# ermongroup/TEOChat

Hardware: AMD Instinct MI355X
Metric: end-to-end tokens/sec (prefill+decode), T=8 frames, LLaMA-2-7B (higher is better)
Workload: dtype bf16; 1 GPU; C3: T=8 frames 224x224 -> CLIP-ViT-L/14 (23 layers) -> mlp2x_gelu -> splice of a 128-token prompt (L=2168) -> LLaMA-2-7B prefill -> 256 forced greedy tokens; value = generated tokens / total time; frames=8, sequence_len=2168, parallelism=dp1 (1 conversation per GPU, no collective), weights=random N(0,0.02^2) at LLaMA-2-7B / ViT-L/14 shapes

## Files before the change

### teochat_amd/_lib.py

```python
import ctypes as C
import os
import threading

HERE = os.path.dirname(os.path.abspath(__file__))
LIB_PATH = os.path.join(HERE, "libteo_hip.so")

TEO_F32, TEO_BF16, TEO_F16 = 0, 1, 2
ACT_NONE, ACT_GELU_ERF, ACT_QUICK_GELU = 0, 1, 2
GEMM_SWIGLU16, GEMM_FORCE_SIMPLE, GEMM_WTILED, GEMM_SWIGLU8, GEMM_F16 = 1, 2, 4, 8, 16
GEMV_W13 = 32
ATTN_FORCE_SIMPLE = 1
INT32_MIN = -(2 ** 31)


class TeoLibraryError(RuntimeError):
    pass


class TeoError(RuntimeError):
    pass


class AttnArgs(C.Structure):
    _fields_ = [("q", C.c_void_p), ("k", C.c_void_p), ("v", C.c_void_p), ("vt", C.c_void_p), ("o", C.c_void_p),
# ... 218 lines not shown
    _fields_ = [("d_next", C.c_void_p), ("n_states", C.c_int), ("vocab", C.c_int), ("d_state", C.c_void_p), ("fallback_token", C.c_longlong)]


_SIGS_GUIDE = {
    "teo_guide_sizeof": (C.c_size_t, []),
    "teo_guide_mask": (C.c_int, [C.c_void_p, C.c_longlong, C.c_int, C.POINTER(Guide), C.c_void_p]),
    "teo_guide_advance": (C.c_int, [C.POINTER(Guide), C.c_void_p, C.c_int, C.c_void_p]),
    "teo_llama_decode_step_guided": (C.c_int, [C.POINTER(LlamaDesc), C.POINTER(DecodeState), C.POINTER(Guide), C.c_void_p, C.c_size_t, C.c_void_p]),
    "teo_llama_decode_graph_create_guided": (C.c_int, [C.POINTER(LlamaDesc), C.POINTER(DecodeState), C.POINTER(Guide), C.c_void_p, C.c_size_t,
                                                       C.c_void_p, C.POINTER(C.c_void_p)]),
    "teo_llama_decode_stream_step_guided": (C.c_int, [C.POINTER(LlamaDesc), C.POINTER(DecodeStreamState), C.POINTER(Guide), C.c_void_p, C.c_size_t,
                                                      C.c_void_p]),
    "teo_llama_decode_stream_graph_create_guided": (C.c_int, [C.POINTER(LlamaDesc), C.POINTER(DecodeStreamState), C.POINTER(Guide), C.c_void_p,
                                                              C.c_size_t, C.c_void_p, C.POINTER(C.c_void_p)]),
}
EXPORTS_GUIDE = tuple(_SIGS_GUIDE.keys())


class Share(C.Structure):
    _fields_ = [("d_lead", C.c_void_p), ("d_rows", C.c_void_p)]


_SIGS_SHARE = {
    "teo_share_sizeof": (C.c_size_t, []),
    "teo_attn_decode_shared": (C.c_int, [C.c_void_p] * 9 + [C.c_int] * 4 + [C.c_float, C.c_int, C.c_int, C.c_longlong, C.c_longlong,
                                                                             C.c_longlong, C.c_void_p, C.c_void_p, C.c_void_p]),
    "teo_attn_decode_chunk": (C.c_int, [C.c_int] * 5 + [C.c_void_p]),
    "teo_llama_decode_stream_step_shared": (C.c_int, [C.POINTER(LlamaDesc), C.POINTER(DecodeStreamState), C.POINTER(Share), C.POINTER(Guide),
                                                      C.c_void_p, C.c_size_t, C.c_void_p]),
    "teo_llama_decode_stream_graph_create_shared": (C.c_int, [C.POINTER(LlamaDesc), C.POINTER(DecodeStreamState), C.POINTER(Share),
                                                              C.POINTER(Guide), C.c_void_p, C.c_size_t, C.c_void_p, C.POINTER(C.c_void_p)]),
}
EXPORTS_SHARE = tuple(_SIGS_SHARE.keys())
_lib = None


def load():
    global _lib
    if _lib is not None:
        return _lib
    import torch
    if not os.path.exists(LIB_PATH):
        raise TeoLibraryError(
            f"{LIB_PATH} not found: the HIP library is required (no CPU fallback). Build it with "
            "`python -c \"import __graft_entry__ as g; g.build()\"` or `make -C teochat_amd/csrc`.")
    try:
        lib = C.CDLL(LIB_PATH)
    except OSError as e:
        raise TeoLibraryError(f"cannot load {LIB_PATH}: {e}") from e
    for name, (res, args) in list(_SIGS.items()) + list(_SIGS_PREFIX.items()) + list(_SIGS_SCORE.items()) + list(_SIGS_GUIDE.items()) \
            + list(_SIGS_SHARE.items()):
        try:
            fn = getattr(lib, name)
        except AttributeError as e:
            raise TeoLibraryError(f"{LIB_PATH} does not export {name}; rebuild it") from e
        fn.restype = res
        fn.argtypes = args
    if lib.teo_version() != ABI_VERSION:
        raise TeoLibraryError(f"ABI version mismatch: library {lib.teo_version()}, binding {ABI_VERSION}; rebuild {LIB_PATH}")
    mirrors = {"teo_vit_desc": VitDesc, "teo_proj_desc": ProjDesc, "teo_llama_desc": LlamaDesc, "teo_decode_state": DecodeState,
               "teo_decode_batch_state": DecodeBatchState, "teo_attn_args": AttnArgs, "teo_verify_state": VerifyState,
               "teo_decode_stream_state": DecodeStreamState}
    for name, cls in mirrors.items():
        want = lib.teo_sizeof(name.encode())
        if want != C.sizeof(cls):
            raise TeoLibraryError(f"struct layout mismatch: {name} is {want} bytes in {LIB_PATH}, {C.sizeof(cls)} in this binding; rebuild")
    if lib.teo_guide_sizeof() != C.sizeof(Guide):
        raise TeoLibraryError(f"struct layout mismatch: teo_guide is {lib.teo_guide_sizeof()} bytes in {LIB_PATH}, {C.sizeof(Guide)} in this binding; rebuild")
    if lib.teo_share_sizeof() != C.sizeof(Share):
        raise TeoLibraryError(f"struct layout mismatch: teo_share is {lib.teo_share_sizeof()} bytes in {LIB_PATH}, {C.sizeof(Share)} in this binding; rebuild")
    _lib = lib
    return lib


class Tune:

    def __init__(self):
        self._lib = load()
        self.ptr = self._lib.teo_tune_create()
        if not self.ptr:
            raise TeoError("teo_tune_create failed")

    def try_set(self, key, value):
        key = key if isinstance(key, bytes) else key.encode()
# ... 75 lines not shown
```

### teochat_amd/csrc/abi.hip

```cpp
#include <stdarg.h>

#include <new>

#include "runtime.h"

namespace teo {

static thread_local char g_err[512] = "";

thread_local const char* g_last_kernel = "";
void note_kernel(const char* name) { g_last_kernel = name; }

void set_error(const char* fmt, ...) {
    va_list ap;
    va_start(ap, fmt);
    vsnprintf(g_err, sizeof(g_err), fmt, ap);
    va_end(ap);
}

int device_cu_count() {
    static int cached[64];
    int dev = 0;
    if (hipGetDevice(&dev) != hipSuccess) return 0;
    if (dev >= 0 && dev < 64 && cached[dev] > 0) return cached[dev];
    hipDeviceProp_t p;
    const int cus = hipGetDeviceProperties(&p, dev) == hipSuccess ? p.multiProcessorCount : 0;
    if (dev >= 0 && dev < 64 && cus > 0) cached[dev] = cus;
    return cus;
}

int lds_attr_once(const void* kernel, int bytes, unsigned long long* mask, const char* what) {
    int dev = 0;
    if (hipGetDevice(&dev) != hipSuccess) dev = 0;
    const unsigned long long bit = 1ull << (dev & 63);
    if (__atomic_load_n(mask, __ATOMIC_RELAXED) & bit) return TEO_OK;
    const hipError_t e = hipFuncSetAttribute(kernel, hipFuncAttributeMaxDynamicSharedMemorySize, bytes);
    if (e != hipSuccess) { set_error("%s: hipFuncSetAttribute(%d bytes of LDS): %s", what, bytes, hipGetErrorString(e)); return TEO_ERR_HIP; }
// ... 681 lines not shown
        if (e != hipSuccess) return hip_fail(e, "hipGraphLaunch");
    }
    return TEO_OK;
}

int teo_graph_destroy(teo_graph* g) {
    if (!g) return TEO_OK;
    if (g->exec) (void)hipGraphExecDestroy(g->exec);
    if (g->graph) (void)hipGraphDestroy(g->graph);
    delete g;
    return TEO_OK;
}

size_t teo_attn_decode_workspace_bytes(int heads, int head_dim, int max_seq, int batch) {
    if (!(heads > 0 && head_dim > 0 && max_seq > 0 && batch > 0)) return 0;
    return attn_decode_ws_bytes(heads, head_dim, max_seq, batch);
}

int teo_attn_decode(const void* q, void* k_cache, void* v_cache, void* vt_cache, const float* rope_cos, const float* rope_sin,
                    void* out, float* partials, const int* d_pos, int max_seq, int heads, int kv_heads, int head_dim, float scale,
                    int dtype, int batch, long long q_stride, long long cache_stride, long long o_stride, teo_stream_t s) {
    ENTER();
    NEED_DT(dtype);
    TEO_CHECK_ARG(batch >= 1 && heads > 0 && kv_heads > 0 && heads % kv_heads == 0 && head_dim > 0 && max_seq > 0,
                  "teo_attn_decode: batch %d heads %d kv_heads %d head_dim %d max_seq %d", batch, heads, kv_heads, head_dim, max_seq);
    NEED(q, "q"); NEED(k_cache, "k_cache"); NEED(v_cache, "v_cache"); NEED(out, "out"); NEED(partials, "partials"); NEED(d_pos, "d_pos");
    TEO_CHECK_ARG((rope_cos == nullptr) == (rope_sin == nullptr), "teo_attn_decode: rope_cos and rope_sin go together");
    AttnBatch bt;
    bt.batch = batch; bt.q_stride = q_stride; bt.cache_stride = cache_stride; bt.o_stride = o_stride;
    return attn_decode(q, k_cache, v_cache, vt_cache, rope_cos, rope_sin, out, partials, d_pos, max_seq, heads, kv_heads, head_dim,
                       scale, dtype, ST(s), bt);
}

size_t teo_attn_verify_workspace_bytes(int heads, int head_dim, int max_seq, int rows) {
    if (!(heads > 0 && head_dim > 0 && max_seq > 0 && rows > 0)) return 0;
    return attn_decode_ws_bytes(heads, head_dim, max_seq, rows);
}

int teo_attn_verify(const void* qkv, void* k_cache, void* v_cache, void* vt_cache, const float* rope_cos, const float* rope_sin,
                    void* out, float* partials, const int* d_pos, int max_seq, int heads, int kv_heads, int head_dim, float scale,
                    int dtype, int rows, long long q_stride, teo_stream_t s) {
    ENTER();
    NEED_DT(dtype);
    TEO_CHECK_ARG(rows >= 1 && rows <= TEO_MAX_DECODE_BATCH && heads > 0 && kv_heads > 0 && heads % kv_heads == 0 && max_seq >= rows,
                  "teo_attn_verify: rows %d (1..%d) heads %d kv_heads %d max_seq %d", rows, TEO_MAX_DECODE_BATCH, heads, kv_heads, max_seq);
    TEO_CHECK_ARG(head_dim > 0, "teo_attn_verify: head_dim %d", head_dim);
    NEED(qkv, "qkv"); NEED(k_cache, "k_cache"); NEED(v_cache, "v_cache"); NEED(out, "out"); NEED(partials, "partials"); NEED(d_pos, "d_pos");
    NEED(rope_cos, "rope_cos"); NEED(rope_sin, "rope_sin");
    TEO_CHECK_ARG(q_stride >= (long long)(heads + 2 * kv_heads) * head_dim && q_stride % (dtype == TEO_F32 ? 4 : 8) == 0,
                  "teo_attn_verify: q_stride %lld (whole [q|k|v] rows, 16-byte aligned)", q_stride);
    return attn_verify(qkv, k_cache, v_cache, vt_cache, rope_cos, rope_sin, out, partials, d_pos, max_seq, heads, kv_heads, head_dim,
                       scale, dtype, rows, q_stride, ST(s));
}

int teo_cross_entropy(const float* logits, long long ld, const long long* labels, float* loss_row, float* out, int rows, int vocab,
                      long long ignore_index, teo_stream_t s) {
    ENTER();
    TEO_CHECK_ARG(rows >= 0 && vocab > 0 && ld >= vocab, "teo_cross_entropy: rows %d vocab %d ld %lld", rows, vocab, ld);
    NEED(out, "out");
    if (rows) { NEED(logits, "logits"); NEED(labels, "labels"); NEED(loss_row, "loss_row"); }
    return cross_entropy(logits, ld, labels, loss_row, out, rows, vocab, ignore_index, ST(s));
}

int teo_preprocess_frames(const unsigned char* src, void* out, int T, int H, int W, int S, const float* mean, const float* stdv,
                          int dtype, teo_stream_t s) {
    ENTER();
// ... 52 lines not shown
```

### teochat_amd/csrc/attention.hip

```cpp
#include "common.h"
#include "ops.h"

namespace teo {

typedef __attribute__((ext_vector_type(8))) short bf16x8;
typedef __attribute__((ext_vector_type(4))) float f32x4;
typedef __attribute__((ext_vector_type(4))) unsigned int u32x4;

template <typename T>
__global__ __launch_bounds__(64) void attn_simple_kernel(teo_attn_args a) {
    extern __shared__ __attribute__((aligned(16))) float sm[];
    float* qs = sm;
    float* sc = sm + a.head_dim;
    const int i = blockIdx.x, h = blockIdx.y, b = blockIdx.z, lane = threadIdx.x;
    const int hk = h / (a.heads / a.kv_heads);
    const int hd = a.head_dim;
    const T* q = (const T*)a.q + b * a.q_bs + h * a.q_hs + (long long)i * a.q_rs;
    const T* k = (const T*)a.k + b * a.k_bs + hk * a.k_hs;
    const T* v = (const T*)a.v + b * a.v_bs + hk * a.v_hs;
    for (int d = lane; d < hd; d += 64) qs[d] = Elem<T>::ld(q + d);
    __syncthreads();
    const int lim = a.causal ? min(a.kv_len, i + (a.kv_len - a.q_len) + 1) : a.kv_len;
    float mx = -INFINITY;
    for (int j = lane; j < lim; j += 64) {
// ... 294 lines not shown
    for (int i = 0; i < SPL; ++i)
        if (DEC_CHUNK >= 64 || lane + 64 * i < DEC_CHUNK) pstrip[wid][lane + 64 * i] = Elem<T>::round(sv[i]);
    float acc[VE];
#pragma unroll
    for (int e = 0; e < VE; ++e) acc[e] = 0.f;
#pragma unroll
    for (int i = 0; i < NI; ++i) {
        const float p = pstrip[wid][wid * KPW + i * RPI + grp];
        if constexpr (ROPE) {
            float vf[VE];
            Cvt16<T>::cvt(vr[i], vf);
            if (kw0 + i * RPI + grp >= pos) {
#pragma unroll
                for (int e = 0; e < VE; ++e) vf[e] = vnew[e];
            }
#pragma unroll
            for (int e = 0; e < VE; ++e) acc[e] = fmaf(p, vf[e], acc[e]);
        } else {
            attn_pv_fma<T>(vr[i], p, acc);
        }
    }
#pragma unroll
    for (int e = 0; e < VE; ++e) acc[e] = cross_group_sum<LPR>(acc[e]);
    if (grp == 0) {
#pragma unroll
        for (int e = 0; e < VE; ++e) obuf[wid][sub * VE + e] = acc[e];
    }
    __syncthreads();
    for (int d = tid; d < HD; d += 256) out[2 + d] = obuf[0][d] + obuf[1][d] + obuf[2][d] + obuf[3][d];
    if (tid == 0) { out[0] = mx; out[1] = sum; }
}

template <typename T>
__device__ __forceinline__ void attn_merge_records(const float* __restrict__ pb, int stride, int nact, int hd_log2, T* __restrict__ o_row,
                                                   float* w , float* red , float* accs ) {
    const int tid = threadIdx.x, lane = tid & 63, wid = tid >> 6;
    const bool on = tid < 512;
    const int hd = 1 << hd_log2;
    const int G = 512 >> hd_log2;
    const int g = on ? tid >> hd_log2 : 0, d = tid & (hd - 1);
    constexpr int NB = 12;
    float v0[NB];
#pragma unroll
    for (int i = 0; i < NB; ++i) v0[i] = pb[(unsigned)(min(g + i * G, nact - 1) * stride + 2 + d)];
    float m0 = -INFINITY, l0 = 0.f;
    if (tid < nact) { m0 = pb[(unsigned)(tid * stride)]; l0 = pb[(unsigned)(tid * stride + 1)]; }
    float M = wave_max(m0);
    if (lane == 0 && on) red[wid] = M;
    __syncthreads();
    M = fmaxf(fmaxf(red[0], red[1]), fmaxf(red[2], red[3]));
    const float w0 = (m0 == -INFINITY) ? 0.f : expf(m0 - M);
    if (tid < 256) w[tid] = w0;
    float L = wave_sum(l0 * w0);
    if (lane == 0 && on) red[8 + wid] = L;
    __syncthreads();
    const float inv = 1.0f / ((red[8] + red[9]) + (red[10] + red[11]));
    float a = 0.f;
#pragma unroll
    for (int i = 0; i < NB; ++i) {
        const float t = v0[i] * w[min(g + i * G, 255)];
        a += (g + i * G < nact) ? t : 0.f;
    }
    for (int s0 = g + NB * G; s0 < nact; s0 += 8 * G) {
        float v[8];
#pragma unroll
        for (int i = 0; i < 8; ++i) v[i] = pb[(unsigned)(min(s0 + i * G, nact - 1) * stride + 2 + d)];
#pragma unroll
        for (int i = 0; i < 8; ++i) {
            const float t = v[i] * w[min(s0 + i * G, 255)];
            a += (s0 + i * G < nact) ? t : 0.f;
        }
    }
    if (on) accs[tid] = a;
    __syncthreads();
    if (on && g == 0) {
        float t = 0.f;
        for (int k = 0; k < G; ++k) t += accs[d + k * hd];
        Elem<T>::st(o_row + d, t * inv);
    }
}

template <typename T>
__global__ __launch_bounds__(512) void attn_decode_combine_kernel(const int* __restrict__ d_pos, const float* __restrict__ part,
                                                                  T* __restrict__ o, int hd_log2, int nsplit, int chunk_log2,
                                                                  long long o_stride) {
    __shared__ float w[256];
    __shared__ float red[16];
    __shared__ float accs[512];
    const int pos = d_pos[blockIdx.y];
    const int h = blockIdx.x;
    const int hd = 1 << hd_log2;
    const int stride = hd + 2;
    part += (long long)blockIdx.y * gridDim.x * nsplit * stride;
    o += (long long)blockIdx.y * o_stride;
    if (pos < 0) {
        if ((int)threadIdx.x < hd) Elem<T>::st(o + h * hd + threadIdx.x, 0.f);
        return;
    }
    const float* pb = part + (long long)h * nsplit * stride;
    const int nact = min(nsplit, (pos + (1 << chunk_log2)) >> chunk_log2);
    attn_merge_records<T>(pb, stride, nact, hd_log2, o + h * hd, w, red, accs);
}

template <typename T, int LPR, int DEC_CHUNK, bool ROPE, int AW_WAVES, bool PROBE = false>
__global__ __launch_bounds__(AW_WAVES * 64) void attn_decode_whole_kernel(const T* __restrict__ q, T* __restrict__ kc, T* __restrict__ vc,
                                                                          T* __restrict__ vtc, const float* __restrict__ cs,
                                                                          const float* __restrict__ sn, T* __restrict__ o,
                                                                          const int* __restrict__ d_pos, int S_max, int heads, int kv_heads,
                                                                          float scale, AttnBatch bt) {
    constexpr int VE = Cvt16<T>::N;
    constexpr int HD = LPR * VE;
    constexpr int RPI = 64 / LPR;
    constexpr int KPQ = DEC_CHUNK / 4;
    constexpr int NI = KPQ / RPI;
    constexpr int SPL = (DEC_CHUNK + 63) / 64;
    constexpr int STRIDE = HD + 2;
    extern __shared__ __attribute__((aligned(16))) float aw_lds[];
    float* sc = aw_lds + (threadIdx.x >> 6) * DEC_CHUNK;
    float* rec = aw_lds + AW_WAVES * DEC_CHUNK;
    {
        const long long bz = blockIdx.y;
        q += bz * bt.q_stride;
        kc += bz * bt.cache_stride;
        vc += bz * bt.cache_stride;
        if (vtc) vtc += bz * bt.cache_stride;
        d_pos += bz;
        o += bz * bt.o_stride;
    }
    const int h = blockIdx.x, tid = threadIdx.x, lane = tid & 63, wid = tid >> 6;
    const int hk = (heads == kv_heads) ? h : h / (heads / kv_heads);
    const int kv_len = *d_pos + 1;
    if (kv_len <= 0) {
        if (!PROBE && tid < HD) Elem<T>::st(o + h * HD + tid, 0.f);
        return;
// ... 142 lines not shown
        }
        mx = wave_max(mx);
        float sum = 0.f;
#pragma unroll
        for (int i = 0; i < SPL; ++i) { sv[i] = expf(sv[i] - mx); sum += sv[i]; }
        sum = wave_sum(sum);
        __builtin_amdgcn_wave_barrier();
#pragma unroll
        for (int i = 0; i < SPL; ++i)
            if (DEC_CHUNK >= 64 || lane + 64 * i < DEC_CHUNK) sc[lane + 64 * i] = Elem<T>::round(sv[i]);
        __builtin_amdgcn_wave_barrier();
        float ot[VE];
        TEO_AW_PV(r0, 0, ot)
        TEO_AW_ISSUE(r0, kb, cn, 0, nlive)
        TEO_AW_PV(r1, 1, ot)
        TEO_AW_ISSUE(r1, kb, cn, 1, nlive)
        TEO_AW_PV(r2, 2, ot)
        TEO_AW_ISSUE(r2, kb, cn, 2, nlive)
        TEO_AW_PV(r3, 3, ot)
        TEO_AW_ISSUE(r3, kb, cn, 3, nlive)
        __builtin_amdgcn_wave_barrier();
        float* rc = rec + (long long)c * STRIDE;
        if (grp == 0) {
#pragma unroll
            for (int e = 0; e < VE; ++e) rc[2 + sub * VE + e] = ot[e];
        }
        if (lane == 0) { rc[0] = mx; rc[1] = sum; }
    }
#undef TEO_AW_ISSUE
#undef TEO_AW_SCORES
#undef TEO_AW_PV
    __syncthreads();
    float* w = rec + (long long)nact * STRIDE;
    attn_merge_records<T>(rec, STRIDE, nact, __builtin_ctz((unsigned)HD), o + h * HD, w, w + 256, w + 272);
}

size_t attn_decode_ws_bytes(int heads, int hd, int S_max, int batch) {
    const int nsplit = cdiv(S_max, 32);
    return (size_t)batch * heads * nsplit * (hd + 2) * sizeof(float);
}

template <typename T, int LPR>
static void attn_decode_launch(const void* q, void* kc, void* vc, void* vtc, const float* cs, const float* sn, void* o,
                               float* part, const int* d_pos, int S_max, int heads, int kv_heads, int hd, float scale,
                               int nsplit, int chunk, bool rope, AttnBatch bt, hipStream_t st) {
    dim3 grid(heads, nsplit, bt.batch);
#define TEO_PART(CH, RP)                                                                                              \
    TEO_KLAUNCH((attn_decode_partial_kernel<T, LPR, CH, RP>), grid, 256, 0, st, d_pos, (T*)kc, (T*)vc, (const T*)q, S_max, heads, kv_heads,      \
                                                                     nsplit, (T*)vtc, cs, sn, part, scale, bt)
#define TEO_PART_R(CH) if (rope) { TEO_PART(CH, true); } else { TEO_PART(CH, false); }
    if constexpr (32 / 4 >= 64 / LPR) {
        if (chunk == 32) { TEO_PART_R(32) } else if (chunk == 64) { TEO_PART_R(64) } else if (chunk == 256) { TEO_PART_R(256) } else { TEO_PART_R(128) }
    } else if constexpr (64 / 4 >= 64 / LPR) {
        if (chunk == 64) { TEO_PART_R(64) } else if (chunk == 256) { TEO_PART_R(256) } else { TEO_PART_R(128) }
    } else {
        if (chunk == 256) { TEO_PART_R(256) } else { TEO_PART_R(128) }
    }
#undef TEO_PART_R
#undef TEO_PART
    prof_bump(1);
    TEO_KLAUNCH((attn_decode_combine_kernel<T>), dim3(heads, bt.batch), 512, 0, st, d_pos, part, (T*)o, __builtin_ctz((unsigned)hd), nsplit,
                __builtin_ctz((unsigned)chunk), bt.o_stride);
    prof_bump(-1);
}

template <typename T, int LPR, int NW>
static int attn_whole_launch_t(const void* q, void* kc, void* vc, void* vtc, const float* cs, const float* sn, void* o, const int* d_pos,
                               int S_max, int heads, int kv_heads, float scale, int chunk, bool rope, AttnBatch bt, size_t lds, hipStream_t st) {
    constexpr int RPI = 64 / LPR;
    dim3 grid(heads, bt.batch);
#define TEO_AW(CH, RP)                                                                                                          \
    {                                                                                                                           \
        static unsigned long long attr_mask = 0;                                                                                \
        if (lds > 48 * 1024) if (int e = lds_attr_once(reinterpret_cast<const void*>(&attn_decode_whole_kernel<T, LPR, CH, RP, NW>), 96 * 1024, &attr_mask, "attn_decode_whole")) return e; \
        TEO_KLAUNCH((attn_decode_whole_kernel<T, LPR, CH, RP, NW>), grid, NW * 64, lds, st, (const T*)q, (T*)kc, (T*)vc, (T*)vtc, cs, sn, \
                    (T*)o, d_pos, S_max, heads, kv_heads, scale, bt);                                                           \
    }
#define TEO_AW_R(CH) { if (rope) TEO_AW(CH, true) else TEO_AW(CH, false) }
    if (chunk == 128) { if constexpr (128 / 4 / RPI >= 1 && 128 / 4 / RPI <= 8) TEO_AW_R(128) else return TEO_ERR_UNSUPPORTED; }
    else if (chunk == 64) { if constexpr (64 / 4 / RPI >= 1 && 64 / 4 / RPI <= 8) TEO_AW_R(64) else return TEO_ERR_UNSUPPORTED; }
    else if (chunk == 32) { if constexpr (32 / 4 / RPI >= 1 && 32 / 4 / RPI <= 8) TEO_AW_R(32) else return TEO_ERR_UNSUPPORTED; }
    else return TEO_ERR_UNSUPPORTED;
#undef TEO_AW_R
#undef TEO_AW
    note_kernel("attn_decode_whole");
    TEO_LAUNCH_CHECK("attn_decode_whole");
    return TEO_OK;
}

static int attn_whole_launch(const void* q, void* kc, void* vc, void* vtc, const float* cs, const float* sn, void* o, const int* d_pos, int S_max,
                             int heads, int kv_heads, int hd, float scale, int chunk, int lpr, int dtype, AttnBatch bt, size_t lds, hipStream_t st) {
    const bool rope = cs != nullptr;
#define TEO_AWL(TT, LL) return attn_whole_launch_t<TT, LL, 8>(q, kc, vc, vtc, cs, sn, o, d_pos, S_max, heads, kv_heads, scale, chunk, rope, bt, lds, st)
    if (dtype == TEO_F32) {
        switch (lpr) { case 4: TEO_AWL(float, 4); case 8: TEO_AWL(float, 8); case 16: TEO_AWL(float, 16); case 32: TEO_AWL(float, 32); default: return TEO_ERR_UNSUPPORTED; }
    }
    if (dtype == TEO_F16) {
        switch (lpr) { case 4: TEO_AWL(f16_t, 4); case 8: TEO_AWL(f16_t, 8); case 16: TEO_AWL(f16_t, 16); case 32: TEO_AWL(f16_t, 32); default: return TEO_ERR_UNSUPPORTED; }
    }
    switch (lpr) { case 4: TEO_AWL(bf16_t, 4); case 8: TEO_AWL(bf16_t, 8); case 16: TEO_AWL(bf16_t, 16); case 32: TEO_AWL(bf16_t, 32); default: return TEO_ERR_UNSUPPORTED; }
#undef TEO_AWL
}

struct AttnDecodePlan {
    int lpr, chunk, nsplit;
    bool ok;
    bool whole;
    int cw;
    size_t lds_whole;
};
static AttnDecodePlan attn_decode_plan(int batch, int heads, int hd, int S_max, int dtype) {
    AttnDecodePlan p;
    int chunk = tune().attn_chunk ? tune().attn_chunk : (batch > 1 ? 128 : 64);
    const int esz = dtype == TEO_F32 ? 4 : 2;
    const int lpr = hd * esz / 16;
    if (chunk / 4 < 64 / lpr) chunk = 4 * (64 / lpr);
    if (chunk != 32 && chunk != 64 && chunk != 128 && chunk != 256) chunk = 128;
    while (chunk < 256 && cdiv(S_max, chunk) > 256) chunk *= 2;
    p.lpr = lpr; p.chunk = chunk; p.nsplit = cdiv(S_max, chunk);
    p.ok = !(p.nsplit > 256 || (hd * esz) % 16 != 0 || (lpr != 2 && lpr != 4 && lpr != 8 && lpr != 16 && lpr != 32));
    p.whole = false; p.cw = 0; p.lds_whole = 0;
    if (!p.ok) return p;
    int cw = tune().attn_chunk ? tune().attn_chunk : 64;
    if (cw / 4 < 64 / lpr) cw = 4 * (64 / lpr);
    while (cw < 128 && cdiv(S_max, cw) > 256) cw *= 2;
    const int nsw = cdiv(S_max, cw);
    const int ni = cw / 4 / (64 / lpr);
    const size_t lds = ((size_t)8 * cw + (size_t)nsw * (hd + 2) + 784) * sizeof(float);
    const int cus = device_cu_count();
    const bool fits = ni >= 1 && ni <= 8 && (hd & (hd - 1)) == 0 && hd <= 256 && lds <= 96 * 1024 && nsw <= 256 && (cw == 32 || cw == 64 || cw == 128);
    const int ncu = cus > 0 ? cus : 256, wgs = batch * heads;
    const bool balanced = wgs >= ncu && (wgs % ncu == 0 || 4 * wgs >= 7 * ncu);
    p.whole = fits && lpr >= 4 && (tune().attn_whole == 2 || (tune().attn_whole == 1 && batch > 1 && balanced));
    p.cw = cw; p.lds_whole = lds;
    return p;
}

int attn_decode(const void* q, void* kc, void* vc, void* vtc, const float* rope_cos, const float* rope_sin, void* o,
                float* part, const int* d_pos, int S_max, int heads, int kv_heads, int hd, float scale, int dtype,
                hipStream_t st, AttnBatch bt) {
    const bool rope = rope_cos != nullptr;
    const AttnDecodePlan pl = attn_decode_plan(bt.batch, heads, hd, S_max, dtype);
    const int lpr = pl.lpr, chunk = pl.chunk, nsplit = pl.nsplit;
    if (!pl.ok) {
        set_error("attn_decode: unsupported head_dim %d / max_seq %d", hd, S_max);
        return TEO_ERR_UNSUPPORTED;
    }
    if (pl.whole) {
        const int rcw = attn_whole_launch(q, kc, vc, vtc, rope_cos, rope_sin, o, d_pos, S_max, heads, kv_heads, hd, scale, pl.cw, lpr, dtype, bt, pl.lds_whole, st);
        if (rcw != TEO_ERR_UNSUPPORTED) return rcw;
    }
#define TEO_DEC(TT, LL) attn_decode_launch<TT, LL>(q, kc, vc, vtc, rope_cos, rope_sin, o, part, d_pos, S_max, heads, kv_heads, hd, scale, nsplit, chunk, rope, bt, st)
    if (dtype == TEO_F32) {
        switch (lpr) { case 2: TEO_DEC(float, 2); break; case 4: TEO_DEC(float, 4); break; case 8: TEO_DEC(float, 8); break;
                       case 16: TEO_DEC(float, 16); break; default: TEO_DEC(float, 32); }
    } else if (dtype == TEO_F16) {
        switch (lpr) { case 2: TEO_DEC(f16_t, 2); break; case 4: TEO_DEC(f16_t, 4); break; case 8: TEO_DEC(f16_t, 8); break;
                       case 16: TEO_DEC(f16_t, 16); break; default: TEO_DEC(f16_t, 32); }
    } else {
        switch (lpr) { case 2: TEO_DEC(bf16_t, 2); break; case 4: TEO_DEC(bf16_t, 4); break; case 8: TEO_DEC(bf16_t, 8); break;
                       case 16: TEO_DEC(bf16_t, 16); break; default: TEO_DEC(bf16_t, 32); }
    }
#undef TEO_DEC
    TEO_LAUNCH_CHECK("attn_decode");
    return TEO_OK;
}


template <typename T, int LPR, int DEC_CHUNK>
__global__ __launch_bounds__(256) void attn_verify_partial_kernel(const int* __restrict__ d_pos, T* __restrict__ kc, T* __restrict__ vc,
                                                                  const T* __restrict__ qkv, int S_max, int heads, int kv_heads, int nsplit,
                                                                  T* __restrict__ vtc, const float* __restrict__ cs,
                                                                  const float* __restrict__ sn, float* __restrict__ part, float scale,
                                                                  int rows, long long q_stride) {
    constexpr int VE = Cvt16<T>::N;
    constexpr int HD = LPR * VE;
    constexpr int RPI = 64 / LPR;
    constexpr int KPW = DEC_CHUNK / 4;
    constexpr int NI = KPW / RPI;
    constexpr int MAXR = TEO_MAX_DECODE_BATCH;
    const int pos = d_pos[0];
    __shared__ float sc[DEC_CHUNK];
    __shared__ float pstrip[4][DEC_CHUNK];
    __shared__ float obuf[4][HD];
    __shared__ uint4 qrot[MAXR][LPR], knew[MAXR][LPR], vnew[MAXR][LPR];
    const int h = blockIdx.x, sp = blockIdx.y, tid = threadIdx.x, lane = tid & 63, wid = tid >> 6;
    const int gq = heads / kv_heads;
    const int hk = h / gq;
    const int c0 = sp * DEC_CHUNK;
    const int nr = min(rows, S_max - pos);
    for (int r = 0; r < rows; ++r) {
        if (r < nr && c0 < pos + r + 1) continue;
        float* out = part + (((long long)r * heads + h) * nsplit + sp) * (HD + 2);
        if (tid == 0) { out[0] = -INFINITY; out[1] = 0.f; }
        for (int d = tid; d < HD; d += 256) out[2 + d] = 0.f;
    }
    if (c0 >= pos + nr) return;
    const int sub = lane % LPR, grp = lane / LPR;
// ... 106 lines not shown
            const float p = pstrip[wid][wid * KPW + i * RPI + grp];
            uint4 vraw = vr[i];
            if (j >= pos) vraw = vnew[min(j, kv_len - 1) - pos][sub];
            float vf[VE];
            Cvt16<T>::cvt(vraw, vf);
#pragma unroll
            for (int e = 0; e < VE; ++e) acc[e] = fmaf(p, vf[e], acc[e]);
        }
#pragma unroll
        for (int e = 0; e < VE; ++e) acc[e] = cross_group_sum<LPR>(acc[e]);
        if (grp == 0) {
#pragma unroll
            for (int e = 0; e < VE; ++e) obuf[wid][sub * VE + e] = acc[e];
        }
        __syncthreads();
        float* out = part + (((long long)r * heads + h) * nsplit + sp) * (HD + 2);
        for (int d = tid; d < HD; d += 256) out[2 + d] = obuf[0][d] + obuf[1][d] + obuf[2][d] + obuf[3][d];
        if (tid == 0) { out[0] = mx; out[1] = sum; }
    }
}

template <typename T>
__global__ __launch_bounds__(512) void attn_verify_combine_kernel(const int* __restrict__ d_pos, const float* __restrict__ part,
                                                                  T* __restrict__ o, int hd_log2, int nsplit, int chunk_log2) {
    __shared__ float w[256];
    __shared__ float red[16];
    __shared__ float accs[512];
    const int pos = d_pos[0] + blockIdx.y;
    const int h = blockIdx.x;
    const int hd = 1 << hd_log2;
    const int stride = hd + 2;
    const float* pb = part + ((long long)blockIdx.y * gridDim.x + h) * nsplit * stride;
    const int nact = min(nsplit, (pos + (1 << chunk_log2)) >> chunk_log2);
    attn_merge_records<T>(pb, stride, nact, hd_log2, o + ((long long)blockIdx.y * gridDim.x + h) * hd, w, red, accs);
}

template <typename T, int LPR>
static void attn_verify_launch(const void* qkv, void* kc, void* vc, void* vtc, const float* cs, const float* sn, void* o, float* part,
                               const int* d_pos, int S_max, int heads, int kv_heads, int hd, float scale, int nsplit, int chunk, int rows,
                               long long q_stride, hipStream_t st) {
    dim3 grid(heads, nsplit);
#define TEO_VPART(CH)                                                                                                  \
    TEO_KLAUNCH((attn_verify_partial_kernel<T, LPR, CH>), grid, 256, 0, st, d_pos, (T*)kc, (T*)vc, (const T*)qkv, S_max, heads, kv_heads, \
                nsplit, (T*)vtc, cs, sn, part, scale, rows, q_stride)
    if constexpr (32 / 4 >= 64 / LPR) {
        if (chunk == 32) { TEO_VPART(32); } else if (chunk == 64) { TEO_VPART(64); } else if (chunk == 256) { TEO_VPART(256); } else { TEO_VPART(128); }
    } else if constexpr (64 / 4 >= 64 / LPR) {
        if (chunk == 64) { TEO_VPART(64); } else if (chunk == 256) { TEO_VPART(256); } else { TEO_VPART(128); }
    } else {
        if (chunk == 256) { TEO_VPART(256); } else { TEO_VPART(128); }
    }
#undef TEO_VPART
    prof_bump(1);
    TEO_KLAUNCH((attn_verify_combine_kernel<T>), dim3(heads, rows), 512, 0, st, d_pos, part, (T*)o, __builtin_ctz((unsigned)hd), nsplit,
                __builtin_ctz((unsigned)chunk));
    prof_bump(-1);
}

int attn_verify(const void* qkv, void* kc, void* vc, void* vtc, const float* rope_cos, const float* rope_sin, void* o, float* part,
                const int* d_pos, int S_max, int heads, int kv_heads, int hd, float scale, int dtype, int rows, long long q_stride,
                hipStream_t st) {
    const AttnDecodePlan pl = attn_decode_plan(rows, heads, hd, S_max, dtype);
    if (!pl.ok) {
        set_error("attn_verify: unsupported head_dim %d / max_seq %d", hd, S_max);
        return TEO_ERR_UNSUPPORTED;
    }
    const int chunk = pl.whole ? pl.cw : pl.chunk;
// ... 252 lines not shown
```

### teochat_amd/csrc/ops.h

```cpp
#pragma once
#include "common.h"
#include "gemm_plan.h"
#include "gemv_plan.h"

struct teo_graph {
    hipGraph_t graph;
    hipGraphExec_t exec;
};

namespace teo {

int layernorm(const void* x, const void* w, const void* b, void* y, int rows, int dim, float eps, int dtype, hipStream_t st);
int rmsnorm(const void* x, const void* w, void* y, int rows, int dim, float eps, int dtype, hipStream_t st);
int vit_embed_ln(const void* patch, const void* cls, const void* pos, const void* w, const void* b, void* out, int T,
                 int NP, int dim, float eps, int dtype, hipStream_t st);

bool gemm_mfma_ok(int M, int N, int K, int lda, int ldc, int dtype, unsigned flags, const void* A, const void* W,
                  const void* bias, const void* res, const void* C);
int gemm(const void* A, const void* W, const void* bias, const void* res, void* C, int M, int N, int K, int lda,
         int ldc, int act, unsigned flags, int dtype, int out_dtype, hipStream_t st, void* sk_ws = nullptr);

int attention(const teo_attn_args* a, int dtype, hipStream_t st);
int attention_flash32(const teo_attn_args& a, hipStream_t st, bool f16 = false);
bool attn_mfma_ok(const teo_attn_args& a, int dtype);
int attn_branches(const teo_attn_args* a, const int* d_branch_start, int dtype, hipStream_t st);
int attention_probs(const teo_attn_args* a, int dtype, void* probs, hipStream_t st);
size_t attn_decode_ws_bytes(int heads, int hd, int S_max, int batch = 1);
struct AttnBatch {
    int batch = 1;
    long long q_stride = 0, cache_stride = 0, o_stride = 0;
};
int attn_decode(const void* q, void* kc, void* vc, void* vtc, const float* rope_cos, const float* rope_sin, void* o,
                float* part, const int* d_pos, int S_max, int heads, int kv_heads, int hd, float scale, int dtype,
                hipStream_t st, AttnBatch bt = AttnBatch());

int attn_decode_shared(const void* q, void* kc, void* vc, void* vtc, const float* rope_cos, const float* rope_sin, void* o, float* part,
                       const int* d_pos, int S_max, int heads, int kv_heads, int hd, float scale, int dtype, hipStream_t st, AttnBatch bt,
                       const int* d_lead, const int* d_rows);
int attn_decode_record_chunk(int batch, int heads, int hd, int S_max, int dtype);

int attn_verify(const void* qkv, void* kc, void* vc, void* vtc, const float* rope_cos, const float* rope_sin, void* o, float* part,
                const int* d_pos, int S_max, int heads, int kv_heads, int hd, float scale, int dtype, int rows, long long q_stride,
                hipStream_t st);

int rope_kv_append(void* qkv, int ld, const int* positions, const float* cs, const float* sn, void* kc, void* vc,
                   void* vtc, int S, int past, const int* d_past, int S_max, int heads, int kv_heads, int hd, int dtype,
                   hipStream_t st);
int vit_value_transpose(const void* qkv, void* vt, int T, int N, int heads, int hd, int ldv, int dtype, hipStream_t st);
int im2col_patches(const void* px, void* cols, int T, int C, int img, int P, int ld, int dtype, hipStream_t st);
int embed_splice(const int* plan, const void* embed, const void* visual, void* out, int rows, int dim, int dtype,
                 hipStream_t st);
int drop_cls(const void* in, void* out, int T, int ntok, int dim, int dtype, hipStream_t st);
int argmax(const float* logits, long long* tok, int rows, int vocab, hipStream_t st);
int decode_advance(const teo_decode_state* s, hipStream_t st);
int sampler_check(int vocab, int top_k, float top_p);
int sample_topk(const float* logits, long long* tok, int vocab, float temperature, int top_k, float top_p, unsigned long long seed,
                unsigned long long draw, hipStream_t st);
int decode_tail(const float* logits, const teo_decode_state* s, const void* embed, void* h, int vocab, int dim, int dtype,
                hipStream_t st, int batch = 1, int out_stride = 0, const void* g0 = nullptr, void* hg = nullptr,
                float* ssq = nullptr, int nparts = 0);
int decode_stream_tail(const float* logits, const teo_decode_state* s, const int* d_limit, const void* embed, void* h, int vocab, int dim,
                       int dtype, hipStream_t st, int batch, int out_stride, const void* g0, void* hg, float* ssq, int nparts);
int verify_tail(const float* logits, const teo_verify_state* s, long long* sel, int vocab, hipStream_t st);
int spec_propose(const long long* hist, const int* d_hist_len, long long* rows_out, int* d_n_draft, int rows, int ngram_max, hipStream_t st);
int embed_token(const long long* tok, const void* embed, void* h, int dim, int dtype, hipStream_t st, int batch = 1);
int embed_token_emit(const long long* tok, const void* embed, void* h, int dim, int dtype, hipStream_t st, int batch,
                     const void* g, void* hg, float* ssq, int nparts);
// ... 67 lines not shown
```

### teochat_amd/csrc/runtime.hip

```cpp
#include <algorithm>
#include <vector>

#include "runtime.h"
#include "guide_dev.h"
#include "share_dev.h"

namespace teo {
struct Carver {
    unsigned char* base;
    size_t off = 0, cap;
    Carver(void* p, size_t c) : base((unsigned char*)p), cap(c) {}
    void* take(size_t bytes) {
        void* r = base ? base + off : nullptr;
        off += align_up(bytes);
        return r;
    }
    bool ok() const { return off <= cap; }
};

struct VitWs {
    void *cols, *patch, *h, *ln, *qkv, *vt, *attn, *mlp, *sk;
    int ldv;
    size_t total;
};
// ... 325 lines not shown
    w.act = c.take((size_t)d->inter * e);
    w.part = (float*)c.take(attn_decode_ws_bytes(d->heads, d->head_dim, d->max_seq));
    w.total = c.off;
    return w;
}

size_t llama_decode_workspace_bytes(const teo_llama_desc* d) { return decode_carve(d, nullptr, 0).total; }

int llama_decode_step(const teo_llama_desc* d, const teo_decode_state* s, void* ws, size_t ws_bytes, hipStream_t st, const teo_guide* g) {
    const DecodeWs w = decode_carve(d, ws, ws_bytes);
    if (w.total > ws_bytes) {
        set_error("teo_llama_decode_step: workspace %zu < %zu", ws_bytes, w.total);
        return TEO_ERR_WORKSPACE;
    }
    const int dt = d->dtype;
    const int D = d->hidden, H = d->heads, Hk = d->kv_heads, hd = d->head_dim, F = d->inter;
    const int QKV = (H + 2 * Hk) * hd;
    const int wf = decode_weight_format(d, linear_forms(d, LIN_QKV).w4 != nullptr);
    for (int l = 0; l < d->layers; ++l) {
        const LinearPick qkv = pick_linear(linear_forms(d, LIN_QKV), wf, l, true), o = pick_linear(linear_forms(d, LIN_O), wf, l, true);
        const LinearPick gu = pick_linear(linear_forms(d, LIN_GATEUP), wf, l, true), dn = pick_linear(linear_forms(d, LIN_DOWN), wf, l, true);
        if (d->rope_in_attn) {
            prof_class(TEO_PROF_QKV);
            TEO_TRY(gemv_w(w.h, qkv.w, qkv.s, qkv.fmt, d->in_norm_w[l], nullptr, w.qkv, QKV, D, d->eps, 0, dt, dt, st));
            prof_class(TEO_PROF_ATTN);
            TEO_TRY(attn_decode(w.qkv, d->k_cache[l], d->v_cache[l], d->vt_cache[l], d->rope_cos, d->rope_sin, w.attn, w.part,
                                s->d_pos, d->max_seq, H, Hk, hd, 1.0f / sqrtf((float)hd), dt, st));
        } else {
            prof_class(TEO_PROF_QKV);
            TEO_TRY(gemv_qkv_rope(w.h, qkv.w, qkv.s, qkv.fmt, d->in_norm_w[l], w.qkv, d->rope_cos, d->rope_sin, s->d_pos, d->k_cache[l],
                                  d->v_cache[l], d->vt_cache[l], d->max_seq, H, Hk, hd, D, d->eps, dt, st));
            prof_class(TEO_PROF_ATTN);
            TEO_TRY(attn_decode(w.qkv, d->k_cache[l], d->v_cache[l], nullptr, nullptr, nullptr, w.attn, w.part, s->d_pos,
                                d->max_seq, H, Hk, hd, 1.0f / sqrtf((float)hd), dt, st));
        }
        prof_class(TEO_PROF_O);
        TEO_TRY(gemv_w(w.attn, o.w, o.s, o.fmt, nullptr, w.h, w.h, D, H * hd, d->eps, 0, dt, dt, st));
        prof_class(TEO_PROF_GATEUP);
        TEO_TRY(gemv_w(w.h, gu.w, gu.s, gu.fmt, d->post_norm_w[l], nullptr, w.act, 2 * F, D, d->eps, TEO_GEMM_SWIGLU16, dt, dt, st));
        prof_class(TEO_PROF_DOWN);
        TEO_TRY(gemv_w(w.act, dn.w, dn.s, dn.fmt, nullptr, w.h, w.h, D, F, d->eps, 0, dt, dt, st));
    }
    {
        const bool h8 = d->lm_head8 != nullptr;
        prof_class(TEO_PROF_LM_HEAD);
        const bool hp = !h8 && d->lm_head_p13 != nullptr;
        TEO_TRY(gemv_w(w.h, h8 ? d->lm_head8 : (hp ? d->lm_head_p13 : d->lm_head), h8 ? d->lm_head_s : nullptr, hp ? (int)GV_W_P13 : (int)h8, d->final_norm_w, nullptr,
                       s->d_logits, d->vocab, D, d->eps, 0, dt, TEO_F32, st));
    }
    prof_class(TEO_PROF_TAIL);
    if (g) return decode_tail_guided(s->d_logits, s, g, d->embed, w.h, d->vocab, D, dt, st);
    return decode_tail(s->d_logits, s, d->embed, w.h, d->vocab, D, dt, st);
}

int llama_decode_step(const teo_llama_desc* d, const teo_decode_state* s, void* ws, size_t ws_bytes, hipStream_t st) {
    return llama_decode_step(d, s, ws, ws_bytes, st, nullptr);
}


struct DecodeBatchWs {
    void *h, *hg, *qkv, *attn, *act;
    float *ssq, *part;
    int nparts;
    size_t total;
};

static DecodeBatchWs decode_batch_carve(const teo_llama_desc* d, int B, void* ws, size_t cap) {
// ... 386 lines not shown
```

Baseline: 405.0 tokens/s.

## Add transposed-V decode attention path split into score and column-tiled PV kernels

Adds a batch-1 decode attention path for 16-bit head_dim 128. A scores kernel writes per-chunk Q·K scores, then a column-tiled kernel reads the transposed V cache, does per-chunk softmax and the PV product, and merges the records per column slice. The non-rope decode step now passes the vt_cache so this path is chosen when the plan allows it. The aim is to spread V reads across more workgroups and read V contiguously, at the cost of an extra launch, a scores round trip through global memory, and redundant per-chunk softmax in each column block.

After: 365.2 tokens/s. -9.8%, worse.

```diff
diff --git a/include/teo_hip_attn_vt.h b/include/teo_hip_attn_vt.h
--- /dev/null
+++ b/include/teo_hip_attn_vt.h
@@ -0,0 +1,16 @@
+#ifndef TEO_HIP_ATTN_VT_H
+#define TEO_HIP_ATTN_VT_H
+
+#include "teo_hip.h"
+
+#ifdef __cplusplus
+extern "C" {
+#endif
+
+int teo_attn_decode_vt(const void* d_q, const void* d_k_cache, const void* d_vt_cache, void* d_out, float* d_partials, const int* d_pos,
+                       int max_seq, int heads, int kv_heads, int head_dim, float scale, int dtype, teo_stream_t stream);
+
+#ifdef __cplusplus
+}
+#endif
+#endif
diff --git a/teochat_amd/_lib.py b/teochat_amd/_lib.py
--- a/teochat_amd/_lib.py
+++ b/teochat_amd/_lib.py
@@ -274,6 +274,11 @@
                                                               C.POINTER(Guide), C.c_void_p, C.c_size_t, C.c_void_p, C.POINTER(C.c_void_p)]),
 }
 EXPORTS_SHARE = tuple(_SIGS_SHARE.keys())
+
+_SIGS_ATTN_VT = {
+    "teo_attn_decode_vt": (C.c_int, [C.c_void_p] * 6 + [C.c_int] * 4 + [C.c_float, C.c_int, C.c_void_p]),
+}
+EXPORTS_ATTN_VT = tuple(_SIGS_ATTN_VT.keys())
 _lib = None
 
 
@@ -291,7 +296,7 @@
     except OSError as e:
         raise TeoLibraryError(f"cannot load {LIB_PATH}: {e}") from e
     for name, (res, args) in list(_SIGS.items()) + list(_SIGS_PREFIX.items()) + list(_SIGS_SCORE.items()) + list(_SIGS_GUIDE.items()) \
-            + list(_SIGS_SHARE.items()):
+            + list(_SIGS_SHARE.items()) + list(_SIGS_ATTN_VT.items()):
         try:
             fn = getattr(lib, name)
         except AttributeError as e:
diff --git a/teochat_amd/csrc/abi.hip b/teochat_amd/csrc/abi.hip
--- a/teochat_amd/csrc/abi.hip
+++ b/teochat_amd/csrc/abi.hip
@@ -3,6 +3,7 @@
 #include <new>
 
 #include "runtime.h"
+#include "../../include/teo_hip_attn_vt.h"
 
 namespace teo {
 
@@ -750,6 +751,16 @@
                        scale, dtype, ST(s), bt);
 }
 
+int teo_attn_decode_vt(const void* q, const void* k_cache, const void* vt_cache, void* out, float* partials, const int* d_pos, int max_seq,
+                       int heads, int kv_heads, int head_dim, float scale, int dtype, teo_stream_t s) {
+    ENTER();
+    NEED_DT(dtype);
+    TEO_CHECK_ARG(heads > 0 && kv_heads > 0 && heads % kv_heads == 0 && head_dim > 0 && max_seq > 0,
+                  "teo_attn_decode_vt: heads %d kv_heads %d head_dim %d max_seq %d", heads, kv_heads, head_dim, max_seq);
+    NEED(q, "q"); NEED(k_cache, "k_cache"); NEED(vt_cache, "vt_cache"); NEED(out, "out"); NEED(partials, "partials"); NEED(d_pos, "d_pos");
+    return attn_decode_vt(q, k_cache, vt_cache, out, partials, d_pos, max_seq, heads, kv_heads, head_dim, scale, dtype, ST(s));
+}
+
 size_t teo_attn_verify_workspace_bytes(int heads, int head_dim, int max_seq, int rows) {
     if (!(heads > 0 && head_dim > 0 && max_seq > 0 && rows > 0)) return 0;
     return attn_decode_ws_bytes(heads, head_dim, max_seq, rows);
diff --git a/teochat_amd/csrc/attention.hip b/teochat_amd/csrc/attention.hip
--- a/teochat_amd/csrc/attention.hip
+++ b/teochat_amd/csrc/attention.hip
@@ -350,13 +350,14 @@
 }
 
 template <typename T>
-__device__ __forceinline__ void attn_merge_records(const float* __restrict__ pb, int stride, int nact, int hd_log2, T* __restrict__ o_row,
-                                                   float* w , float* red , float* accs ) {
+__device__ __forceinline__ void attn_merge_records(const float* __restrict__ pb, int stride, int nact, int hd_log2, int nc_log2,
+                                                   T* __restrict__ o_row, float* w , float* red , float* accs ) {
     const int tid = threadIdx.x, lane = tid & 63, wid = tid >> 6;
     const bool on = tid < 512;
-    const int hd = 1 << hd_log2;
+    const int nc = 1 << nc_log2;
     const int G = 512 >> hd_log2;
-    const int g = on ? tid >> hd_log2 : 0, d = tid & (hd - 1);
+    const bool col = tid < (G << nc_log2);
+    const int g = col ? tid >> nc_log2 : 0, d = tid & (nc - 1);
     constexpr int NB = 12;
     float v0[NB];
 #pragma unroll
@@ -389,11 +390,11 @@
             a += (s0 + i * G < nact) ? t : 0.f;
         }
     }
-    if (on) accs[tid] = a;
+    if (col) accs[tid] = a;
     __syncthreads();
-    if (on && g == 0) {
+    if (col && g == 0) {
         float t = 0.f;
-        for (int k = 0; k < G; ++k) t += accs[d + k * hd];
+        for (int k = 0; k < G; ++k) t += accs[d + k * nc];
         Elem<T>::st(o_row + d, t * inv);
     }
 }
@@ -417,7 +418,151 @@
     }
     const float* pb = part + (long long)h * nsplit * stride;
     const int nact = min(nsplit, (pos + (1 << chunk_log2)) >> chunk_log2);
-    attn_merge_records<T>(pb, stride, nact, hd_log2, o + h * hd, w, red, accs);
+    attn_merge_records<T>(pb, stride, nact, hd_log2, hd_log2, o + h * hd, w, red, accs);
+}
+
+template <typename T>
+__global__ __launch_bounds__(256) void attn_decode_scores_kernel(const int* __restrict__ d_pos, const T* __restrict__ kc,
+                                                                 const T* __restrict__ q, int S_max, int heads, int kv_heads, int nsplit,
+                                                                 float* __restrict__ scores, float scale) {
+    constexpr int LPR = 16, DEC_CHUNK = 64;
+    constexpr int VE = Cvt16<T>::N;
+    constexpr int HD = LPR * VE;
+    constexpr int RPI = 64 / LPR, KPW = DEC_CHUNK / 4, NI = KPW / RPI;
+    static_assert(sizeof(T) == 2 && HD == 128, "attn_decode_scores_kernel: 16-bit elements, head_dim 128");
+    const int kv_len = d_pos[0] + 1;
+    const int h = blockIdx.x, sp = blockIdx.y, tid = threadIdx.x, lane = tid & 63, wid = tid >> 6;
+    const int hk = (heads == kv_heads) ? h : h / (heads / kv_heads);
+    const int c0 = sp * DEC_CHUNK;
+    if (c0 >= kv_len) return;
+    const int sub = lane % LPR, grp = lane / LPR;
+    const T* kb = kc + (long long)hk * S_max * HD + sub * VE;
+    const int kw0 = c0 + wid * KPW;
+    uint4 kr[NI];
+#pragma unroll
+    for (int i = 0; i < NI; ++i) {
+        const int j = min(kw0 + i * RPI + grp, kv_len - 1);
+        kr[i] = ld_kv(kb + (long long)j * HD);
+    }
+    float qf[VE];
+    Cvt16<T>::cvt(*reinterpret_cast<const uint4*>(q + h * HD + sub * VE), qf);
+    const uint4 qpk = Cvt16<T>::pack(qf);
+    float* out = scores + ((long long)h * nsplit + sp) * DEC_CHUNK;
+#pragma unroll
+    for (int i = 0; i < NI; ++i) {
+        const uint4 kraw = kr[i];
+        const int j = kw0 + i * RPI + grp;
+        float s = 0.f;
+        s = attn_dot2(kraw.x, qpk.x, s); s = attn_dot2(kraw.y, qpk.y, s);
+        s = attn_dot2(kraw.z, qpk.z, s); s = attn_dot2(kraw.w, qpk.w, s);
+        s = group_sum<LPR>(s);
+        if (sub == 0) out[j - c0] = (j < kv_len) ? s * scale : -INFINITY;
+    }
+}
+
+template <typename T, bool HI>
+__device__ __forceinline__ float attn_pv_fma1(unsigned wd, float p, float acc) {
+    if constexpr (IsF16<T>::v) {
+        if constexpr (HI) asm("v_fma_mix_f32 %0, %1, %2, %0 op_sel:[1,0,0] op_sel_hi:[1,0,0]" : "+v"(acc) : "v"(wd), "v"(p));
+        else asm("v_fma_mix_f32 %0, %1, %2, %0 op_sel_hi:[1,0,0]" : "+v"(acc) : "v"(wd), "v"(p));
+        return acc;
+    } else {
+        return fmaf(p, __uint_as_float(HI ? (wd & 0xffff0000u) : (wd << 16)), acc);
+    }
+}
+
+#ifndef TEO_ATTN_VT_COLS
+#define TEO_ATTN_VT_COLS 8
+#endif
+constexpr int ATTN_VT_COLS = TEO_ATTN_VT_COLS;
+
+template <typename T, int NC>
+__global__ __launch_bounds__(512) void attn_decode_vt_kernel(const int* __restrict__ d_pos, const T* __restrict__ vtc,
+                                                             const float* __restrict__ scores, T* __restrict__ o, int S_max, int heads,
+                                                             int kv_heads, int nsplit) {
+    constexpr int HD = 128, CH = 64;
+    constexpr int CPP = 512 / NC;
+    constexpr int SPW = CPP / 8;
+    constexpr int PST = CH + 1;
+    constexpr int STRIDE = NC + 2;
+    static_assert(sizeof(T) == 2 && (NC == 4 || NC == 8 || NC == 16), "attn_decode_vt_kernel: 16-bit elements, 4 / 8 / 16 columns");
+    __shared__ float ps[CPP * PST];
+    __shared__ float rec[256 * STRIDE];
+    __shared__ float w[256];
+    __shared__ float red[16];
+    __shared__ float accs[512];
+    const int pos = d_pos[0];
+    const int h = blockIdx.y, col0 = blockIdx.x * NC, tid = threadIdx.x, lane = tid & 63, wid = tid >> 6;
+    if (pos < 0) {
+        if (tid < NC) Elem<T>::st(o + h * HD + col0 + tid, 0.f);
+        return;
+    }
+    const int kv_len = pos + 1;
+    const int nact = min(nsplit, (pos + CH) / CH);
+    const int hk = (heads == kv_heads) ? h : h / (heads / kv_heads);
+    const int cl = tid / CPP, slot = tid % CPP;
+    const float* sb = scores + (long long)h * nsplit * CH;
+    const T* vrow = vtc + ((long long)hk * HD + col0 + cl) * S_max;
+    for (int cb = 0; cb < nact; cb += CPP) {
+        float sv[SPW];
+#pragma unroll
+        for (int i = 0; i < SPW; ++i) sv[i] = sb[(unsigned)(min(cb + wid + 8 * i, nact - 1) * CH + lane)];
+        __builtin_amdgcn_sched_barrier(0);
+        const int c = cb + slot;
+        const bool live = c < nact;
+        unsigned vw[32];
+#pragma unroll
+        for (int t = 0; t < 8; ++t) {
+            const uint4 r = ld_kv(vrow + (unsigned)(min(c, nact - 1) * CH + t * 8));
+            vw[4 * t] = r.x; vw[4 * t + 1] = r.y; vw[4 * t + 2] = r.z; vw[4 * t + 3] = r.w;
+        }
+        __builtin_amdgcn_sched_barrier(0);
+#pragma unroll
+        for (int i = 0; i < SPW; ++i) {
+            const int cc = cb + wid + 8 * i;
+            float mx = -INFINITY;
+            mx = fmaxf(mx, sv[i]);
+            mx = wave_max(mx);
+            float sum = 0.f;
+            const float e = expf(sv[i] - mx);
+            sum += e;
+            sum = wave_sum(sum);
+            if (cc < nact) {
+                ps[(wid + 8 * i) * PST + lane] = Elem<T>::round(e);
+                if (lane == 0) { rec[cc * STRIDE] = mx; rec[cc * STRIDE + 1] = sum; }
+            }
+        }
+        __syncthreads();
+        if (live) {
+            const int nvalid = kv_len - c * CH;
+            if (nvalid < CH) {
+#pragma unroll
+                for (int m = 0; m < 32; ++m)
+                    vw[m] &= (2 * m < nvalid ? 0x0000ffffu : 0u) | (2 * m + 1 < nvalid ? 0xffff0000u : 0u);
+            }
+            const float* pp = ps + slot * PST;
+            float r = 0.f;
+#pragma unroll
+            for (int wq = 0; wq < 4; ++wq) {
+                float a[4];
+#pragma unroll
+                for (int g = 0; g < 4; ++g) {
+                    float acc = 0.f;
+#pragma unroll
+                    for (int i = 0; i < 4; ++i) {
+                        const int k = 16 * wq + 4 * i + g;
+                        acc = (k & 1) ? attn_pv_fma1<T, true>(vw[k >> 1], pp[k], acc) : attn_pv_fma1<T, false>(vw[k >> 1], pp[k], acc);
+                    }
+                    a[g] = acc;
+                }
+                const float qs = (a[0] + a[1]) + (a[2] + a[3]);
+                r = wq == 0 ? qs : r + qs;
+            }
+            rec[c * STRIDE + 2 + cl] = r;
+        }
+        __syncthreads();
+    }
+    attn_merge_records<T>(rec, STRIDE, nact, __builtin_ctz((unsigned)HD), __builtin_ctz((unsigned)NC), o + h * HD + col0, w, red, accs);
 }
 
 template <typename T, int LPR, int DEC_CHUNK, bool ROPE, int AW_WAVES, bool PROBE = false>
@@ -626,7 +771,7 @@
 #undef TEO_AW_PV
     __syncthreads();
     float* w = rec + (long long)nact * STRIDE;
-    attn_merge_records<T>(rec, STRIDE, nact, __builtin_ctz((unsigned)HD), o + h * HD, w, w + 256, w + 272);
+    attn_merge_records<T>(rec, STRIDE, nact, __builtin_ctz((unsigned)HD), __builtin_ctz((unsigned)HD), o + h * HD, w, w + 256, w + 272);
 }
 
 size_t attn_decode_ws_bytes(int heads, int hd, int S_max, int batch) {
@@ -658,6 +803,17 @@
     prof_bump(-1);
 }
 
+template <typename T>
+static void attn_decode_vt_launch(const void* q, const void* kc, const void* vt, void* o, float* part, const int* d_pos, int S_max, int heads,
+                                  int kv_heads, float scale, int nsplit, hipStream_t st) {
+    TEO_KLAUNCH((attn_decode_scores_kernel<T>), dim3(heads, nsplit), 256, 0, st, d_pos, (const T*)kc, (const T*)q, S_max, heads, kv_heads, nsplit,
+                part, scale);
+    prof_bump(1);
+    TEO_KLAUNCH((attn_decode_vt_kernel<T, ATTN_VT_COLS>), dim3(128 / ATTN_VT_COLS, heads), 512, 0, st, d_pos, (const T*)vt, part, (T*)o, S_max,
+                heads, kv_heads, nsplit);
+    prof_bump(-1);
+}
+
 template <typename T, int LPR, int NW>
 static int attn_whole_launch_t(const void* q, void* kc, void* vc, void* vtc, const float* cs, const float* sn, void* o, const int* d_pos,
                                int S_max, int heads, int kv_heads, float scale, int chunk, bool rope, AttnBatch bt, size_t lds, hipStream_t st) {
@@ -702,9 +858,11 @@
     bool whole;
     int cw;
     size_t lds_whole;
+    bool vt;
 };
-static AttnDecodePlan attn_decode_plan(int batch, int heads, int hd, int S_max, int dtype) {
+static AttnDecodePlan attn_decode_plan(int batch, int heads, int hd, int S_max, int dtype, const void* vt_stream = nullptr, bool rope = false) {
     AttnDecodePlan p;
+    p.vt = false;
     int chunk = tune().attn_chunk ? tune().attn_chunk : (batch > 1 ? 128 : 64);
     const int esz = dtype == TEO_F32 ? 4 : 2;
     const int lpr = hd * esz / 16;
@@ -727,14 +885,16 @@
     const bool balanced = wgs >= ncu && (wgs % ncu == 0 || 4 * wgs >= 7 * ncu);
     p.whole = fits && lpr >= 4 && (tune().attn_whole == 2 || (tune().attn_whole == 1 && batch > 1 && balanced));
     p.cw = cw; p.lds_whole = lds;
+    p.vt = !p.whole && batch == 1 && esz == 2 && hd == 128 && chunk == 64 && S_max % 64 == 0 && vt_stream != nullptr &&
+           (reinterpret_cast<uintptr_t>(vt_stream) & 15) == 0 && !rope;
     return p;
 }
 
 int attn_decode(const void* q, void* kc, void* vc, void* vtc, const float* rope_cos, const float* rope_sin, void* o,
                 float* part, const int* d_pos, int S_max, int heads, int kv_heads, int hd, float scale, int dtype,
-                hipStream_t st, AttnBatch bt) {
+                hipStream_t st, AttnBatch bt, const void* vt_stream) {
     const bool rope = rope_cos != nullptr;
-    const AttnDecodePlan pl = attn_decode_plan(bt.batch, heads, hd, S_max, dtype);
+    const AttnDecodePlan pl = attn_decode_plan(bt.batch, heads, hd, S_max, dtype, vt_stream, rope);
     const int lpr = pl.lpr, chunk = pl.chunk, nsplit = pl.nsplit;
     if (!pl.ok) {
         set_error("attn_decode: unsupported head_dim %d / max_seq %d", hd, S_max);
@@ -743,6 +903,12 @@
     if (pl.whole) {
         const int rcw = attn_whole_launch(q, kc, vc, vtc, rope_cos, rope_sin, o, d_pos, S_max, heads, kv_heads, hd, scale, pl.cw, lpr, dtype, bt, pl.lds_whole, st);
         if (rcw != TEO_ERR_UNSUPPORTED) return rcw;
+    }
+    if (pl.vt) {
+        if (dtype == TEO_F16) attn_decode_vt_launch<f16_t>(q, kc, vt_stream, o, part, d_pos, S_max, heads, kv_heads, scale, nsplit, st);
+        else attn_decode_vt_launch<bf16_t>(q, kc, vt_stream, o, part, d_pos, S_max, heads, kv_heads, scale, nsplit, st);
+        TEO_LAUNCH_CHECK("attn_decode");
+        return TEO_OK;
     }
 #define TEO_DEC(TT, LL) attn_decode_launch<TT, LL>(q, kc, vc, vtc, rope_cos, rope_sin, o, part, d_pos, S_max, heads, kv_heads, hd, scale, nsplit, chunk, rope, bt, st)
     if (dtype == TEO_F32) {
@@ -758,6 +924,17 @@
 #undef TEO_DEC
     TEO_LAUNCH_CHECK("attn_decode");
     return TEO_OK;
+}
+
+int attn_decode_vt(const void* q, const void* kc, const void* vt, void* o, float* part, const int* d_pos, int S_max, int heads, int kv_heads,
+                   int hd, float scale, int dtype, hipStream_t st) {
+    const AttnDecodePlan pl = attn_decode_plan(1, heads, hd, S_max, dtype, vt, false);
+    if (!pl.ok || !pl.vt) {
+        set_error("attn_decode_vt: the shape runs the split + combine pair (head_dim %d, max_seq %d, dtype %d)", hd, S_max, dtype);
+        return TEO_ERR_UNSUPPORTED;
+    }
+    return attn_decode(q, const_cast<void*>(kc), nullptr, nullptr, nullptr, nullptr, o, part, d_pos, S_max, heads, kv_heads, hd, scale, dtype, st,
+                       AttnBatch(), vt);
 }
 
 
@@ -930,7 +1107,7 @@
     const int stride = hd + 2;
     const float* pb = part + ((long long)blockIdx.y * gridDim.x + h) * nsplit * stride;
     const int nact = min(nsplit, (pos + (1 << chunk_log2)) >> chunk_log2);
-    attn_merge_records<T>(pb, stride, nact, hd_log2, o + ((long long)blockIdx.y * gridDim.x + h) * hd, w, red, accs);
+    attn_merge_records<T>(pb, stride, nact, hd_log2, hd_log2, o + ((long long)blockIdx.y * gridDim.x + h) * hd, w, red, accs);
 }
 
 template <typename T, int LPR>
diff --git a/teochat_amd/csrc/ops.h b/teochat_amd/csrc/ops.h
--- a/teochat_amd/csrc/ops.h
+++ b/teochat_amd/csrc/ops.h
@@ -32,7 +32,9 @@
 };
 int attn_decode(const void* q, void* kc, void* vc, void* vtc, const float* rope_cos, const float* rope_sin, void* o,
                 float* part, const int* d_pos, int S_max, int heads, int kv_heads, int hd, float scale, int dtype,
-                hipStream_t st, AttnBatch bt = AttnBatch());
+                hipStream_t st, AttnBatch bt = AttnBatch(), const void* vt_stream = nullptr);
+int attn_decode_vt(const void* q, const void* kc, const void* vt, void* o, float* part, const int* d_pos, int S_max, int heads, int kv_heads,
+                   int hd, float scale, int dtype, hipStream_t st);
 
 int attn_decode_shared(const void* q, void* kc, void* vc, void* vtc, const float* rope_cos, const float* rope_sin, void* o, float* part,
                        const int* d_pos, int S_max, int heads, int kv_heads, int hd, float scale, int dtype, hipStream_t st, AttnBatch bt,
diff --git a/teochat_amd/csrc/runtime.hip b/teochat_amd/csrc/runtime.hip
--- a/teochat_amd/csrc/runtime.hip
+++ b/teochat_amd/csrc/runtime.hip
@@ -381,7 +381,7 @@
                                   d->v_cache[l], d->vt_cache[l], d->max_seq, H, Hk, hd, D, d->eps, dt, st));
             prof_class(TEO_PROF_ATTN);
             TEO_TRY(attn_decode(w.qkv, d->k_cache[l], d->v_cache[l], nullptr, nullptr, nullptr, w.attn, w.part, s->d_pos,
-                                d->max_seq, H, Hk, hd, 1.0f / sqrtf((float)hd), dt, st));
+                                d->max_seq, H, Hk, hd, 1.0f / sqrtf((float)hd), dt, st, AttnBatch(), d->vt_cache[l]));
         }
         prof_class(TEO_PROF_O);
         TEO_TRY(gemv_w(w.attn, o.w, o.s, o.fmt, nullptr, w.h, w.h, D, H * hd, d->eps, 0, dt, dt, st));
```
